# HpWang-whu/RoReg

Measured on AMD Instinct MI355X. Metric: pair-registrations/sec, higher is better.
Workload: dtype f32 (every f32 operand enters the fp16 matrix cores as hi + lo fp16 under a per-keypoint power-of-two block scale: <= 22 significant bits relative to a CONSERVATIVE per-keypoint bound -- measured on the extractor: the bound sits 2^2..2^6 above the keypoint's true coefficient maximum (config.f16x2_sc

## Files before the change

### include/roreg_hip.h

```cpp
#ifndef ROREG_HIP_H
#define ROREG_HIP_H

#include <stdint.h>
#include <stddef.h>

#ifdef __cplusplus
extern "C" {
#endif

#define ROREG_ABI_VERSION 6
int roreg_abi_version(void);
const char *roreg_last_error(void);

int roreg_set_group_tables(const int32_t *P_host, const int32_t *Nei_host, const double *R_host);

size_t roreg_group_conv_packed_size(int Cin, int Cout, int KS);
int roreg_group_conv_pack_weights(const float *W_host , int Cin, int Cout, int KS,
                                  float *wpack_host );
size_t roreg_group_conv_workspace_size(int B, int Cin, int Cout, int Lin, int Lout, int KS);
int roreg_group_conv(const float *x, const float *wpack, const float *bias,
                     const float *bn_scale, const float *bn_shift, const float *residual,
                     float *out, const int32_t *gather,
                     int B, int Cin, int Cout, int Lin, int Lout, int KS,
                     float *workspace, size_t workspace_floats, void *stream);
// ... 215 lines not shown
size_t roreg_irrep_gemm_tiles(int O, int B, int32_t *tiles_host);
size_t roreg_irrep_gemm_tiles_m(int O, int B, int tile_m , int32_t *tiles_host);
int roreg_irrep_gemm(const float *const *X, float *const *Out, const float *const *Add, const float *const *Wpack, int C, int O, int B,
                     const int32_t *tiles_dev, int n_tiles, void *stream);
int roreg_irrep_gemm_split(const float *const *X, float *const *Out, const float *const *Add, const void *const *Wsplit, int C, int O, int B,
                           const int32_t *tiles_dev, int n_tiles, void *stream);
int roreg_irrep_gemm_f16x2(const float *const *X, float *const *Out, const float *const *Add, const void *const *Wsplit2,
                           const float *x_bound_dev, int w_exp, const float *next_u_dev, const float *next_v_dev, float *out_bound_dev,
                           int C, int O, int B, const int32_t *tiles_dev, int n_tiles,
                           int tile_m ,
                           int x_planes , void *stream);
int roreg_gemm_persistent(int on);
int roreg_gemm_thin(int on);
int roreg_irrep_gemm_f16x2_rows(const float *const *X, float *T3r, const void *const *Wsplit2, const float *x_bound_dev, int w_exp, int C, int B, void *stream);
int roreg_gf_finish(const float *T3r, const float *x, const float *b_out, const float *role_scale , const float *role_shift ,
                    float *eqv, float *inv, float *role_out , float *eqv_ft, int B, void *stream);
int roreg_gf_finish_route(int on);
int roreg_row_bound(const void *x_spatial, int x_bf16 , const float *bn_scale, const float *bn_shift,
                    float *bound_out, int B, int C, void *stream);
int roreg_ft_nonlin(const float *Xin , const float *x_spatial, const float *bias,
                    const float *bias2, const float *bn_scale, const float *bn_shift, const float *resid_spatial,
                    float *Xout , float *out_spatial ,
                    const int32_t *g_map ,
                    int Lout , int Lvalid,
                    int B, int C, int split ,
                    const float *out_bound ,
                    float *out_rowmax ,
                    int spatial_bf16 ,
                    int out_planes ,
                    void *stream);
int roreg_ft_nonlin_packed(const float *Xin, const float *bias, const float *bn_scale, const float *bn_shift, uint32_t *out_words,
                           const int32_t *g_map, int Lout, int Lvalid, int B, int C, const float *out_bound, float *raw_col, int raw_g,
                           void *stream);
int roreg_ft_nonlin_gathered(const uint64_t *rows , const int64_t *dr , int feat_bf16, const float *bn_scale ,
                             const float *bn_shift, float *Xout, int B, const float *out_bound , int out_planes, void *stream);

typedef struct roreg_icp_grid_desc {
    double origin[3];
    double edge;
    int32_t dims[3];
    int32_t n;
    int64_t cells;
    int64_t reserved;
} roreg_icp_grid_desc;
size_t roreg_icp_grid_size(const double *lo_host, const double *hi_host, int n, double max_dist, roreg_icp_grid_desc *desc_host,
                           size_t *workspace_bytes);
int roreg_icp_grid_build(const float *points, const roreg_icp_grid_desc *desc_host, void *grid, void *workspace, size_t workspace_bytes,
                         void *stream);
typedef struct roreg_icp_task {
    const void *tgt_grid;
    const void *src_grid;
    const double *T0;
    int32_t n_src;
    int32_t slot0;
} roreg_icp_task;
size_t roreg_icp_batch_workspace(int n_tasks, long long total_slots);
int roreg_icp_batch(const roreg_icp_task *tasks, int n_tasks, const int32_t *work, int n_work, long long total_slots, double max_dist,
                    int max_iter, double tol_deg, double tol_t, double *T_out, int32_t *iters_out, int32_t *inliers_out, double *rmse_out,
                    int32_t *status_out, int32_t *assign_out, double *stats_out, void *workspace, size_t workspace_bytes, void *stream);

int roreg_icp_normals(const void *grid, double radius, int min_neighbors, double *out, void *stream);
typedef struct roreg_icp_plane_task {
    const void *tgt_grid;
    const void *src_grid;
    const double *tgt_normals;
    const double *T0;
// ... 155 lines not shown
```

### roreg_amd/_abi.py

```python
import ctypes
from ctypes import c_int, c_void_p, c_size_t, c_double, c_float, c_char_p

import numpy as np

ABI_VERSION = 6

_P = c_void_p
PROTOTYPES = {
    'roreg_abi_version': (c_int, []),
    'roreg_last_error': (c_char_p, []),
    'roreg_set_group_tables': (c_int, [_P, _P, _P]),
    'roreg_group_conv_packed_size': (c_size_t, [c_int, c_int, c_int]),
    'roreg_group_conv_pack_weights': (c_int, [_P, c_int, c_int, c_int, _P]),
    'roreg_group_conv_workspace_size': (c_size_t, [c_int, c_int, c_int, c_int, c_int, c_int]),
    'roreg_group_conv': (c_int, [_P, _P, _P, _P, _P, _P, _P, _P, c_int, c_int, c_int, c_int, c_int, c_int, _P, c_size_t, _P]),
    'roreg_group_conv_split': (c_int, [_P, _P, _P, _P, _P, _P, _P, _P, c_int, c_int, c_int, c_int, c_int, c_int, c_int, _P]),
    'roreg_group_conv_f16x2': (c_int, [_P, _P, c_int, _P, _P, _P, c_float, c_float, _P, _P, _P, _P, _P, c_int, c_int, c_int, c_int, c_int, c_int, c_int, _P]),
    'roreg_group_conv_f16x2_packed': (c_int, [_P, _P, c_int, _P, _P, _P, _P, _P, _P, c_int, c_int, c_int, c_int, c_int, c_int, c_int, _P]),
    'roreg_dense_f16x2': (c_int, [_P, _P, c_int, _P, _P, _P, c_float, c_float, _P, _P, c_int, _P, _P, c_int, c_int, c_int, _P]),
    'roreg_dense_split': (c_int, [_P, _P, _P, _P, _P, _P, c_int, _P, c_int, c_int, c_int, _P]),
    'roreg_gf_finalize': (c_int, [_P, _P, c_int, _P, c_int, _P]),
    'roreg_det_score': (c_int, [_P, _P, c_int, _P]),
    'roreg_inv_descriptor': (c_int, [_P, c_int, _P, c_int, _P]),
    'roreg_nn_search': (c_int, [_P, _P, c_int, _P, _P, c_int, c_int, _P, _P, _P, _P]),
# ... 84 lines not shown
    'roreg_pg_optimize_batch': (c_int, [_P, _P, c_int, _P, _P, _P, _P, _P, _P, _P, _P, _P, _P, _P, c_int, c_int, _P, _P, _P, _P, _P, _P, _P, _P, _P, _P, _P, c_size_t, _P]),
    'roreg_sparse_map_workspace': (c_size_t, [c_int]),
    'roreg_sparse_stride_map': (c_int, [_P, c_int, c_int, _P, c_int, _P, _P, _P, _P, _P, c_size_t, _P]),
    'roreg_sparse_kernel_map': (c_int, [_P, c_int, _P, c_int, c_int, c_int, _P, _P, _P, c_size_t, _P]),
    'roreg_sparse_conv': (c_int, [_P, c_int, c_int, c_int, _P, c_int, c_int, _P, c_int, _P, _P, _P, c_int, c_int, _P, c_int, _P]),
    'roreg_sparse_l2norm': (c_int, [_P, c_int, c_int, _P, _P]),
    'roreg_group_feature_assemble': (c_int, [_P, c_int, c_int, _P, _P, c_int, c_int, c_int, _P, c_int, _P, _P]),
    'roreg_sc2_workspace': (c_size_t, [ctypes.c_longlong, ctypes.c_longlong, ctypes.c_longlong, _P]),
    'roreg_sc2_hypotheses_batch': (c_int, [_P, c_int, ctypes.c_longlong, ctypes.c_longlong, ctypes.c_longlong, c_int, c_int, c_double, c_int, _P, _P, _P, _P, c_size_t, _P]),
    'roreg_fpfh_spfh_workspace': (c_size_t, [c_int]),
    'roreg_fpfh_features_workspace': (c_size_t, [c_int]),
    'roreg_fpfh_orient': (c_int, [_P, c_int, _P, _P, _P, _P]),
    'roreg_fpfh_spfh': (c_int, [_P, c_int, _P, c_double, _P, _P, _P, c_size_t, _P]),
    'roreg_fpfh_features': (c_int, [_P, c_int, _P, _P, c_double, _P, _P, _P, c_size_t, _P]),
    'roreg_fpfh_match_workspace': (c_size_t, [ctypes.c_longlong, c_int, _P]),
    'roreg_fpfh_match_batch': (c_int, [_P, c_int, c_int, c_int, ctypes.c_longlong, _P, _P, _P, _P, _P, _P, _P, c_size_t, _P]),
    'roreg_grid_knn': (c_int, [_P, c_int, c_int, c_double, _P, _P, c_int, _P, _P, _P, _P, _P]),
    'roreg_cluster_workspace': (c_size_t, [c_int]),
    'roreg_grid_dbscan': (c_int, [_P, c_int, c_double, c_int, _P, _P, _P, _P, _P, c_size_t, _P]),
    'roreg_profile_enable': (c_int, [c_int]),
    'roreg_profile_read': (c_int, [c_int, _P, _P]),
    'roreg_set_fourier_tables': (c_int, [_P]),
    'roreg_mt_shuffle_prefix': (c_int, [_P, c_int, _P, c_int, c_int, _P, c_int]),
    'roreg_mt_stream_shuffle_prefix': (c_int, [_P, _P, _P, c_int, c_int, _P]),
    'roreg_irrep_gemm_tiles': (c_size_t, [c_int, c_int, _P]),
    'roreg_irrep_gemm_tiles_m': (c_size_t, [c_int, c_int, c_int, _P]),
    'roreg_irrep_gemm': (c_int, [_P, _P, _P, _P, c_int, c_int, c_int, _P, c_int, _P]),
    'roreg_irrep_gemm_split': (c_int, [_P, _P, _P, _P, c_int, c_int, c_int, _P, c_int, _P]),
    'roreg_irrep_gemm_f16x2': (c_int, [_P, _P, _P, _P, _P, c_int, _P, _P, _P, c_int, c_int, c_int, _P, c_int, c_int, c_int, _P]),
    'roreg_row_bound': (c_int, [_P, c_int, _P, _P, _P, c_int, c_int, _P]),
    'roreg_ft_nonlin': (c_int, [_P, _P, _P, _P, _P, _P, _P, _P, _P, _P, c_int, c_int, c_int, c_int, c_int, _P, _P, c_int, c_int, _P]),
    'roreg_ft_nonlin_packed': (c_int, [_P, _P, _P, _P, _P, _P, c_int, c_int, c_int, c_int, _P, _P, c_int, _P]),
    'roreg_ft_nonlin_gathered': (c_int, [_P, _P, c_int, _P, _P, _P, c_int, _P, c_int, _P]),
}


_RANSAC_TASK = np.dtype([('keys0', np.uint64), ('keys1', np.uint64), ('matches', np.uint64), ('w', np.uint64), ('Trans', np.uint64),
                         ('hyp_rows', np.uint64), ('M', np.int32), ('H', np.int32), ('koff', np.int64)])

_MATCH_TASK = np.dtype([('desc0', np.uint64), ('desc1', np.uint64), ('rows0', np.uint64), ('rows1', np.uint64), ('m0', np.int32), ('m1', np.int32)])

_GATHER_TASK = np.dtype([('src', np.uint64), ('rows', np.uint64), ('dst', np.uint64), ('n', np.int32), ('pad', np.int32)])

_LT_TASK = np.dtype([('before0', np.uint64), ('before1', np.uint64), ('after0', np.uint64), ('after1', np.uint64), ('keys0', np.uint64),
                     ('keys1', np.uint64), ('matches', np.uint64), ('sel', np.uint64), ('n', np.int32), ('pad', np.int32), ('off', np.int64),
                     ('coef0', np.uint64), ('coef1', np.uint64)])

_ICP_GRID_DESC = np.dtype([('origin', np.float64, 3), ('edge', np.float64), ('dims', np.int32, 3), ('n', np.int32), ('cells', np.int64),
                           ('reserved', np.int64)])

_ICP_TASK = np.dtype([('tgt_grid', np.uint64), ('src_grid', np.uint64), ('T0', np.uint64), ('n_src', np.int32), ('slot0', np.int32)])

_ICP_PLANE_TASK = np.dtype([('tgt_grid', np.uint64), ('src_grid', np.uint64), ('tgt_normals', np.uint64), ('T0', np.uint64), ('n_src', np.int32),
                            ('slot0', np.int32)])

_ICP_GICP_TASK = np.dtype([('tgt_grid', np.uint64), ('src_grid', np.uint64), ('tgt_normals', np.uint64), ('src_normals', np.uint64), ('T0', np.uint64),
                           ('epsilon', np.float64), ('n_src', np.int32), ('slot0', np.int32)])

_ICP_LOSS = {'huber': 1, 'cauchy': 2, 'gm': 3, 'tukey': 4}
_ICP_PLANE_ROBUST_TASK = np.dtype(_ICP_PLANE_TASK.descr + [('scale', np.float64), ('loss', np.int32), ('reserved', np.int32)])
_ICP_GICP_ROBUST_TASK = np.dtype(_ICP_GICP_TASK.descr + [('scale', np.float64), ('loss', np.int32), ('reserved', np.int32)])
assert _ICP_PLANE_ROBUST_TASK.itemsize == 56 and _ICP_GICP_ROBUST_TASK.itemsize == 72

_PG_GRAPH = np.dtype([('node0', np.int32), ('n_nodes', np.int32), ('edge0', np.int32), ('n_edges', np.int32), ('act0', np.int32), ('n_act', np.int32),
                      ('anchor', np.int32), ('reserved0', np.int32), ('h0', np.int64), ('tau', np.float64), ('lambda0', np.float64),
                      ('tol_t', np.float64), ('tol_rot', np.float64), ('tol_cost', np.float64), ('reserved1', np.float64)])
# ... 8 lines not shown
```

### roreg_amd/_hip_fourier.py

```python
import os
from ctypes import c_void_p

import numpy as np
import torch

from . import hip as _core
from .hip import HipError, _check, _feat, _ptr, _stream, lib

__all__ = ['DenseSplitLayer', 'IRREP_DIMS', 'IRREP_OFFSETS', '_bf16_split3', '_keypoint_of_columns', '_ptr_array', '_res_ptr', '_tile_cache', 'bf16_split3_frags', 'bf16_split3_pack', 'bound_exp', 'coef_pitch', 'coef_size', 'coef_views', 'dense_split', 'ensure_fourier', 'f16_scale_exp', 'f16_split2_frags', 'f16_split2_pack', 'frag_pack', 'ft_nonlin', 'ft_nonlin_gathered', 'ft_nonlin_packed', 'gemm_persistent', 'gemm_thin', 'gf_finish', 'gf_finish_rows', 'gf_finish_usable', 'group_conv_split_pack', 'irrep_gemm', 'irrep_gemm_rows', 'next_bound', 'next_bound_spatial', 'pack_coefs_f16x2', 'row_bound', 'unpack_coefs_f16x2', 'words_to_planes']


_fourier_ready = False
IRREP_DIMS = (1, 3, 3, 4, 5)
IRREP_OFFSETS = (0, 1, 10, 19, 35, 60)


def ensure_fourier():
    global _fourier_ready
    if not _fourier_ready:
        from .fourier import group_fourier
        F = np.ascontiguousarray(group_fourier().F, np.float32)
        _check(lib().roreg_set_fourier_tables(F.ctypes.data), 'roreg_set_fourier_tables')
        _fourier_ready = True


def _ptr_array(views):
    arr = (c_void_p * 5)(*[c_void_p(v.data_ptr()) for v in views])
    return arr


def coef_pitch(B):
    return (int(B) + 31) // 32 * 32


def coef_size(C, B):
    return 60 * C * coef_pitch(B)


def coef_views(buf, C, B):
    Bp = coef_pitch(B)
    return [buf[IRREP_OFFSETS[r] * C * Bp:IRREP_OFFSETS[r + 1] * C * Bp].view(IRREP_DIMS[r] * C, IRREP_DIMS[r] * Bp) for r in range(5)]

# ... 159 lines not shown
        o.copy_(w.view(torch.float32))
    return out, bound


def words_to_planes(X_words, C, B):
    w = X_words.contiguous().view(torch.int32).view(-1, 2, 16)
    hi = (w & 0xffff).to(torch.int16).transpose(1, 2); lo = (w >> 16).to(torch.int16).transpose(1, 2)
    return torch.cat([hi.reshape(-1, 32), lo.reshape(-1, 32)], 1).contiguous().view(torch.float32).view(-1)


def unpack_coefs_f16x2(X_words, bound, C, B):
    Bp = coef_pitch(B)
    e = bound_exp(bound)
    out = torch.empty_like(X_words)
    for r, (v, o) in enumerate(zip(coef_views(X_words, C, B), coef_views(out, C, B))):
        kp = _keypoint_of_columns(IRREP_DIMS[r], Bp)
        w = v.view(torch.int32)
        hi = (w & 0xffff).to(torch.int16).view(torch.float16).float()
        lo = (w >> 16).to(torch.int16).view(torch.float16).float()
        o.copy_(torch.ldexp(hi + lo, -e[kp][None, :]))
    return out


def next_bound_spatial(bn, bias):
    scale, shift = bn
    sc = scale.detach().double().abs().cpu(); sh = shift.detach().double().abs().cpu()
    b = bias.detach().double().cpu()
    k = 1.0 + 2.0 ** -9
    u = (np.sqrt(60.0) * k) * sc
    v = k * (sc * b.abs() + sh) + 1e-30
    return u.float().cuda().contiguous(), v.float().cuda().contiguous()


def ft_nonlin_packed(B, C, coef_in, bias, bn, out_bound, g_map=None, Lout=60, Lvalid=60, raw_g=None):
    ensure_fourier()
    dev = coef_in.device
    if coef_in.numel() != coef_size(C, B) or out_bound.numel() != coef_pitch(B):
        raise HipError('ft_nonlin_packed: coef_in / out_bound sizes')
    words = torch.empty((B, C, Lout if g_map is not None else 60), dtype=torch.int32, device=dev)
    raw = torch.empty((B, C), dtype=torch.float32, device=dev) if raw_g is not None else None
    scale, shift = bn if bn is not None else (None, None)
    _check(lib().roreg_ft_nonlin_packed(_ptr(coef_in, torch.float32), _ptr(bias), _ptr(scale), _ptr(shift), _ptr(words), _ptr(g_map, torch.int32),
                                        int(Lout), int(Lvalid), B, C, _ptr(out_bound, torch.float32), _ptr(raw), int(raw_g or 0), _stream()),
           'roreg_ft_nonlin_packed')
    return words, raw


def next_bound(bn, bias, bias2=None):
    scale, shift = bn
    sc = scale.detach().double().abs().cpu(); sh = shift.detach().double().abs().cpu()
    b = bias.detach().double().cpu() + (bias2.detach().double().cpu() if bias2 is not None else 0.0)
    k = 1.0 + 2.0 ** -9
    u = (60.0 * k) * sc
    v = (np.sqrt(60.0) * k) * (sc * b.abs() + sh) + 1e-30
    return u.float().cuda().contiguous(), v.float().cuda().contiguous()


def ft_nonlin(B, C, coef_in=None, x_spatial=None, bias=None, bias2=None, bn=None, resid_spatial=None, spatial_out=False,
              g_map=None, Lout=60, Lvalid=60, split=False, out_bound=None, want_rowmax=False, planes=False):
    ensure_fourier()
    dev = (coef_in if coef_in is not None else x_spatial).device
    if spatial_out:
        out = torch.empty((B, C, Lout if g_map is not None else 60), dtype=torch.float32, device=dev); xout = None; osp = _ptr(out)
    else:
        out = torch.empty(coef_size(C, B), dtype=torch.float32, device=dev); xout = _ptr(out); osp = None
    scale, shift = bn if bn is not None else (None, None)
    if want_rowmax and not spatial_out:
        raise HipError('ft_nonlin: want_rowmax goes with spatial_out')
    amax = torch.zeros(B, dtype=torch.float32, device=dev) if want_rowmax else None
# ... 123 lines not shown
```

### roreg_amd/csrc/fourier.hip

```cpp
#include "common.h"
#include "primitives.h"
#include <algorithm>
#include <atomic>
#include <cmath>
#include <cstdlib>
#include <type_traits>
#include <utility>
#include <vector>

namespace {

constexpr int NIRR = 5;

struct GemmDescs {
    const float *X[NIRR];
    float *Out[NIRR];
    const float *Add[NIRR];
    const float4 *W[NIRR];
    int K[NIRR], M[NIRR], Mpad[NIRR], N[NIRR];
};

__device__ __forceinline__ void lds_dma16(const void *src, void *dst) {
    __builtin_amdgcn_global_load_lds((const __attribute__((address_space(1))) void *)src, (__attribute__((address_space(3))) void *)dst, 16, 0, 0);
}
// ... 1984 lines not shown
                    unsigned *dst = reinterpret_cast<unsigned *>(const_cast<char *>(slot_ptr(ic, p.Xout, c, tb)));
                    if (kPS.kind[S] != 2 || h == 0) __builtin_nontemporal_store(word, dst);
                });
            } else {
                const int tb = tbi;
                static_for<32>([&](auto ic) {
                    constexpr int S = decltype(ic)::value, t = S / 16, r = S % 16;
                    float *dst = reinterpret_cast<float *>(const_cast<char *>(slot_ptr(ic, p.Xout, c, tb)));
                    if (kPS.kind[S] != 2 || h == 0) __builtin_nontemporal_store(o[t][r], dst);
                });
            }
        }
    };
    if (wave_global < n_tiles) {
        const int last = wave_global + ((n_tiles - 1 - wave_global) / n_waves) * n_waves;
        float cb[NCV + 1];
        GDesc da{0u, 0u, 0}, db{0u, 0u, 0};
        if constexpr (GATHER) {
            da = load_desc(wave_global);
            db = load_desc(min(wave_global + n_waves, last));
            load_rows_gathered(wave_global, da, cn);
        } else {
            load_coefs(wave_global, cn);
        }
        __builtin_amdgcn_s_waitcnt(0x0F70);
        for (int tile = wave_global; tile <= last; tile += 2 * n_waves) {
            const int t1 = min(tile + n_waves, last), t2 = min(tile + 2 * n_waves, last), t3 = min(tile + 3 * n_waves, last);
            process(tile, t1, cn, cb, t2, db, da);
            process(t1, t2, cb, cn, t3, da, db);
        }
    }
}

#undef OFF_OF
#undef OFF_Q

struct GfFinishParams {
    const float *T3r;
    const float *x;
    const float *b_out;
    const float *role_scale, *role_shift;
    float *eqv, *inv, *role_out, *eqv_ft;
    const f16x8 *A1h, *A2h;
    int f_exp, B;
};

__global__ __launch_bounds__(256, 2) void gf_finish_kernel(GfFinishParams p) {
    constexpr int NA = 4 * 2 * 2 * 64 * 4;
    extern __shared__ __attribute__((aligned(16))) float gf_smem[];
    float *sA1 = gf_smem, *sA2 = gf_smem + NA, *sT = gf_smem + 2 * NA, *sRole = sT + 4 * 32 * 65;
    const int lane = threadIdx.x & 63, jn = lane & 31, h = lane >> 5;
    {
        const float *g1 = reinterpret_cast<const float *>(p.A1h), *g2 = reinterpret_cast<const float *>(p.A2h);
        for (int i = threadIdx.x; i < NA; i += 256) { sA1[i] = g1[i]; sA2[i] = g2[i]; }
        if (threadIdx.x < 128) sRole[threadIdx.x] = p.role_scale ? (threadIdx.x < 64 ? p.role_scale[threadIdx.x] : p.role_shift[threadIdx.x - 64]) : 0.f;
    }
    __syncthreads();
    const f16x8 *sA1h = reinterpret_cast<const f16x8 *>(sA1), *sA2h = reinterpret_cast<const f16x8 *>(sA2);
    const int wave_global = __builtin_amdgcn_readfirstlane((blockIdx.x * 256 + threadIdx.x) >> 6);
    const int n_waves = gridDim.x * 4;
    const int B = p.B;
    const bool act = lane < ROREG_G;
    const float bo = p.b_out[jn] + 0.f;
    float *ti = sT + (threadIdx.x >> 6) * (32 * 65);

    auto load = [&](int b, float (&cv)[32], float (&xv)[32]) {
// ... 138 lines not shown
                if constexpr (kPS.qb[S] < ROREG_G) ti[jn * 65 + kPS.qb[S]] = o[S / 16][S % 16];
            });
        }
        ROREG_LDS_DONE();
        float *fo = p.eqv_ft + (size_t)b * (ROREG_F * ROREG_G) + lane;
#pragma unroll
        for (int c8 = 0; c8 < 4; ++c8) {
            float tv[8];
#pragma unroll
            for (int q = 0; q < 8; ++q) tv[q] = ti[(c8 * 8 + q) * 65 + lane];
#pragma unroll
            for (int q = 0; q < 8; ++q)
                if (act) fo[(c8 * 8 + q) * ROREG_G] = tv[q];
        }
        ROREG_LDS_DONE();
    };
#undef ROREG_LDS_DONE
    if (wave_global < B) {
        const int last = wave_global + ((B - 1 - wave_global) / n_waves) * n_waves;
        float ca[32], xa[32], cb[32], xb[32];
        load(wave_global, ca, xa);
        __builtin_amdgcn_s_waitcnt(0x0F70);
        for (int b = wave_global; b <= last; b += 2 * n_waves) {
            const int b1 = min(b + n_waves, last), b2 = min(b + 2 * n_waves, last);
            process(b, b1, ca, xa, cb, xb);
            process(b1, b2, cb, xb, ca, xa);
        }
    }
}

float *g_A1 = nullptr, *g_A2 = nullptr;
uint16_t *g_A1s = nullptr, *g_A2s = nullptr, *g_A1h = nullptr, *g_A2h = nullptr;
int g_f_exp = 0;

}

extern "C" int roreg_set_fourier_tables(const float *F_host ) {
    ROREG_REQUIRE(F_host, "roreg_set_fourier_tables: null table");
    static float A1[30 * 2 * 64], A2[32 * 2 * 64];
    for (int s = 0; s < 30; ++s)
        for (int tile = 0; tile < 2; ++tile)
            for (int lane = 0; lane < 64; ++lane) {
                const int qq = 2 * s + (lane >> 5), g = tile * 32 + (lane & 31);
                A1[(s * 2 + tile) * 64 + lane] = g < 60 ? F_host[qq * 60 + g] : 0.f;
            }
    for (int t = 0; t < 2; ++t)
        for (int r = 0; r < 16; ++r)
            for (int tile = 0; tile < 2; ++tile)
                for (int lane = 0; lane < 64; ++lane) {
                    const int qq = slot_out_q(tile * 32 + (lane & 31)), g = cd_row32(r, lane >> 5, t * 32);
                    A2[((t * 16 + r) * 2 + tile) * 64 + lane] = (qq < 60 && g < 60) ? F_host[qq * 60 + g] : 0.f;
                }
    if (!g_A1) {
        if (hipMalloc(&g_A1, sizeof(A1)) != hipSuccess || hipMalloc(&g_A2, sizeof(A2)) != hipSuccess) {
            roreg::set_error("roreg_set_fourier_tables: hipMalloc failed");
            return 1;
        }
    }
    if (hipMemcpy(g_A1, A1, sizeof(A1), hipMemcpyHostToDevice) != hipSuccess || hipMemcpy(g_A2, A2, sizeof(A2), hipMemcpyHostToDevice) != hipSuccess) {
        roreg::set_error("roreg_set_fourier_tables: hipMemcpy failed");
        return 1;
    }
    static uint16_t A1s[4 * 2 * 3 * 64 * 8], A2s[4 * 2 * 3 * 64 * 8];
    auto split3_host = [](float x, uint16_t out[3]) {
        float rem = x;
        for (int sp = 0; sp < 3; ++sp) {
// ... 38 lines not shown
    int fex = 0;
    (void)std::frexp(fmx, &fex);
    g_f_exp = fmx > 0.f ? 14 - fex : 0;
    auto f2h = [](float x) -> uint16_t {
        _Float16 hv = (_Float16)x;
        uint16_t b; memcpy(&b, &hv, 2);
        return b;
    };
    auto h2f = [](uint16_t b) -> float { _Float16 hv; memcpy(&hv, &b, 2); return (float)hv; };
    for (int st = 0; st < 4; ++st)
        for (int tile = 0; tile < 2; ++tile)
            for (int lane = 0; lane < 64; ++lane)
                for (int e = 0; e < 8; ++e) {
                    const int j = lane & 31, h = lane >> 5;
                    const int q1 = 16 * st + 8 * h + e, g1 = tile * 32 + j;
                    const float f1 = (q1 < 60 && g1 < 60) ? std::ldexp(F_host[q1 * 60 + g1], g_f_exp) : 0.f;
                    const int r = 8 * (st & 1) + e, q2 = slot_out_q(tile * 32 + j), g2 = cd_row32(r, h, 32 * (st >> 1));
                    const float f2 = (q2 < 60 && g2 < 60) ? std::ldexp(F_host[q2 * 60 + g2], g_f_exp) : 0.f;
                    const uint16_t h1 = f2h(f1), h2 = f2h(f2);
                    const size_t hi_at = ((((size_t)st * 2 + tile) * 2 + 0) * 64 + lane) * 8 + e, lo_at = hi_at + 64 * 8;
                    A1h[hi_at] = h1; A1h[lo_at] = f2h(f1 - h2f(h1));
                    A2h[hi_at] = h2; A2h[lo_at] = f2h(f2 - h2f(h2));
                }
    if (!g_A1h) {
        if (hipMalloc(&g_A1h, sizeof(A1h)) != hipSuccess || hipMalloc(&g_A2h, sizeof(A2h)) != hipSuccess) {
            roreg::set_error("roreg_set_fourier_tables: hipMalloc failed");
            return 1;
        }
    }
    if (hipMemcpy(g_A1h, A1h, sizeof(A1h), hipMemcpyHostToDevice) != hipSuccess || hipMemcpy(g_A2h, A2h, sizeof(A2h), hipMemcpyHostToDevice) != hipSuccess) {
        roreg::set_error("roreg_set_fourier_tables: hipMemcpy failed");
        return 1;
    }
    return 0;
}

extern "C" size_t roreg_irrep_gemm_tiles_m(int O, int B, int tile_m, int32_t *tiles_host);
extern "C" size_t roreg_irrep_gemm_tiles(int O, int B, int32_t *tiles_host ) { return roreg_irrep_gemm_tiles_m(O, B, 128, tiles_host); }

extern "C" size_t roreg_irrep_gemm_tiles_m(int O, int B, int tile_m , int32_t *tiles_host) {
    static const int dims[5] = {1, 3, 3, 4, 5};
    struct Block { int r, mg, ng, cost; };
    std::vector<Block> blocks;
    for (int r = 4; r >= 0; --r) {
        const int d = dims[r];
        const int mts = round_up(d * O, tile_m) / tile_m, nts = (d * B + 255) / 256;
        for (int ng = 0; ng * 8 < nts; ++ng)
            for (int mg = 0; mg * 8 < mts; ++mg) {
                const int a = std::min(8, mts - mg * 8), b = std::min(8, nts - ng * 8);
                blocks.push_back({r, mg, ng, a * b * d});
            }
    }
    std::stable_sort(blocks.begin(), blocks.end(), [](const Block &x, const Block &y) { return x.cost > y.cost; });
    std::vector<std::vector<int>> stream(8);
    long long load[8] = {0, 0, 0, 0, 0, 0, 0, 0};
    for (const Block &bk : blocks) {
        int k = 0;
        for (int q = 1; q < 8; ++q)
            if (load[q] < load[k]) k = q;
        load[k] += bk.cost;
        const int d = dims[bk.r];
        const int mts = round_up(d * O, tile_m) / tile_m, nts = (d * B + 255) / 256;
        for (int nt = bk.ng * 8; nt < std::min(nts, bk.ng * 8 + 8); ++nt)
            for (int mt = bk.mg * 8; mt < std::min(mts, bk.mg * 8 + 8); ++mt) {
                stream[k].push_back(bk.r); stream[k].push_back(mt); stream[k].push_back(nt);
            }
// ... 231 lines not shown
    p.bias = bias; p.bias2 = bias2; p.bn_scale = bn_scale; p.bn_shift = bn_shift; p.A1 = g_A1; p.A2 = g_A2;
    p.A1s = reinterpret_cast<const bf16x8 *>(g_A1s); p.A2s = reinterpret_cast<const bf16x8 *>(g_A2s); p.out_bound = out_bound; p.out_rowmax = out_rowmax; p.x_bf16 = spatial_bf16;
    p.A1h = reinterpret_cast<const f16x8 *>(g_A1h); p.A2h = reinterpret_cast<const f16x8 *>(g_A2h); p.f_exp = g_f_exp;
    p.B = B; p.Bp = (B + 31) / 32 * 32; p.C = C; p.tiles_per_c = (B + 31) / 32;
    p.out_planes = out_planes;
    ROREG_REQUIRE((unsigned long long)C * p.Bp * 20ull < (1ull << 32), "roreg_ft_nonlin: C * round_up(B, 32) must stay below 2^32 / 20 (32-bit lane offsets)");
    ROREG_REQUIRE(!out_planes || (split == 2 && Xout), "roreg_ft_nonlin: out_planes is a layout of the fp16 x 2 coefficient output");
    const long long n_tiles = (long long)C * p.tiles_per_c;
    hipStream_t s = roreg::as_stream(stream);
    roreg::ProfScope prof(roreg::PROF_FT_NONLIN, s);
    const bool in_sp = x_spatial != nullptr, out_sp = out_spatial != nullptr;
    if (in_sp && out_sp) { roreg::set_error("roreg_ft_nonlin: spatial -> spatial is not a transform"); return 2; }
    ROREG_REQUIRE(split != 2 || out_sp || out_bound, "roreg_ft_nonlin: split = 2 writes the coefficients as fp16 hi/lo pairs and needs out_bound");
    ROREG_REQUIRE(!spatial_bf16 || in_sp || resid_spatial, "roreg_ft_nonlin: spatial_bf16 refers to x_spatial / resid_spatial");
    ROREG_REQUIRE(!out_rowmax || out_sp, "roreg_ft_nonlin: out_rowmax goes with a group-domain output");
    ROREG_REQUIRE(split >= 0 && split <= 2, "roreg_ft_nonlin: split must be 0 (f32 MFMA), 1 (bf16 x 3) or 2 (fp16 x 2)");
    if (split == 2) {
        if (in_sp) launch_ft<ft_nonlin_kernel<true, false, 2, 4, 1>>(p, n_tiles, s);
        else if (!out_sp) launch_ft<ft_nonlin_kernel<false, false, 2, 4, 1>>(p, n_tiles, s);
        else launch_ft<ft_nonlin_kernel<false, true, 2, 4, 1>>(p, n_tiles, s);
    } else if (split == 1) {
        if (in_sp) launch_ft<ft_nonlin_kernel<true, false, 3, 4, 1>>(p, n_tiles, s);
        else if (!out_sp) launch_ft<ft_nonlin_kernel<false, false, 3, 4, 1>>(p, n_tiles, s);
        else launch_ft<ft_nonlin_kernel<false, true, 3, 4, 1>>(p, n_tiles, s);
    } else {
        if (in_sp) launch_ft<ft_nonlin_kernel<true, false, 0, 4, 1>>(p, n_tiles, s);
        else if (!out_sp) launch_ft<ft_nonlin_kernel<false, false, 0, 4, 1>>(p, n_tiles, s);
        else launch_ft<ft_nonlin_kernel<false, true, 0, 4, 1>>(p, n_tiles, s);
    }
    ROREG_CHECK_LAUNCH("roreg_ft_nonlin");
    return 0;
}

extern "C" int roreg_ft_nonlin_packed(const float *Xin, const float *bias, const float *bn_scale, const float *bn_shift, uint32_t *out_words,
                                      const int32_t *g_map, int Lout, int Lvalid, int B, int C, const float *out_bound, float *raw_col, int raw_g,
                                      void *stream) {
    ROREG_REQUIRE(g_A1 && g_A2, "roreg_ft_nonlin_packed: roreg_set_fourier_tables has not been called");
    ROREG_REQUIRE(Xin && out_words && out_bound && B > 0 && C > 0 && C <= 512 && (bn_scale == nullptr) == (bn_shift == nullptr), "roreg_ft_nonlin_packed: bad arguments");
    ROREG_REQUIRE(!g_map || (Lout >= Lvalid && Lvalid > 0 && Lout <= 64), "roreg_ft_nonlin_packed: bad Lout/Lvalid");
    ROREG_REQUIRE(!raw_col || (raw_g >= 0 && raw_g < ROREG_G), "roreg_ft_nonlin_packed: raw_g out of range");
    NonlinParams p;
    memset(&p, 0, sizeof(p));
    p.Xin = Xin; p.out_spatial = reinterpret_cast<float *>(out_words);
    p.g_map = g_map; p.Lout = g_map ? Lout : ROREG_G; p.Lvalid = g_map ? Lvalid : ROREG_G;
    p.bias = bias; p.bn_scale = bn_scale; p.bn_shift = bn_shift; p.A1 = g_A1; p.A2 = g_A2;
    p.A1s = reinterpret_cast<const bf16x8 *>(g_A1s); p.A2s = reinterpret_cast<const bf16x8 *>(g_A2s);
    p.A1h = reinterpret_cast<const f16x8 *>(g_A1h); p.A2h = reinterpret_cast<const f16x8 *>(g_A2h); p.f_exp = g_f_exp;
    p.out_bound = out_bound; p.sp_pack = 1; p.raw_col = raw_col; p.raw_g = raw_g;
    p.B = B; p.Bp = (B + 31) / 32 * 32; p.C = C; p.tiles_per_c = (B + 31) / 32;
    ROREG_REQUIRE((unsigned long long)C * p.Bp * 20ull < (1ull << 32), "roreg_ft_nonlin_packed: C * round_up(B, 32) must stay below 2^32 / 20 (32-bit lane offsets)");
    hipStream_t s = roreg::as_stream(stream);
    roreg::ProfScope prof(roreg::PROF_FT_NONLIN, s);
    launch_ft<ft_nonlin_kernel<false, true, 2, 4, 1>>(p, (long long)C * p.tiles_per_c, s);
    ROREG_CHECK_LAUNCH("roreg_ft_nonlin_packed");
    return 0;
}

extern "C" int roreg_ft_nonlin_gathered(const uint64_t *rows, const int64_t *dr, int feat_bf16, const float *bn_scale, const float *bn_shift, float *Xout,
                                        int B, const float *out_bound, int out_planes, void *stream) {
    ROREG_REQUIRE(g_A1 && g_A2, "roreg_ft_nonlin_gathered: roreg_set_fourier_tables has not been called");
    ROREG_REQUIRE(roreg::group_tables().ready, "roreg_ft_nonlin_gathered: group tables not set");
    ROREG_REQUIRE(rows && dr && Xout && out_bound && B > 0 && (bn_scale == nullptr) == (bn_shift == nullptr), "roreg_ft_nonlin_gathered: bad arguments");
    constexpr int C = 4 * ROREG_F;
    ROREG_REQUIRE((long long)60 * C * B < (1ll << 40), "roreg_ft_nonlin_gathered: tensor too large");
    NonlinParams p;
    memset(&p, 0, sizeof(p));
    p.Xout = Xout; p.Lout = ROREG_G; p.Lvalid = ROREG_G;
    p.bn_scale = bn_scale; p.bn_shift = bn_shift; p.A1 = g_A1; p.A2 = g_A2;
    p.A1s = reinterpret_cast<const bf16x8 *>(g_A1s); p.A2s = reinterpret_cast<const bf16x8 *>(g_A2s);
    p.A1h = reinterpret_cast<const f16x8 *>(g_A1h); p.A2h = reinterpret_cast<const f16x8 *>(g_A2h); p.f_exp = g_f_exp;
    p.out_bound = out_bound; p.x_bf16 = feat_bf16; p.out_planes = out_planes;
    p.g_rows = reinterpret_cast<const roreg::LtRow *>(rows); p.g_dr = dr; p.g_P8 = roreg::group_tables().P8;
    p.B = B; p.Bp = (B + 31) / 32 * 32; p.C = C; p.tiles_per_c = (B + 31) / 32;
    ROREG_REQUIRE((unsigned long long)C * p.Bp * 20ull < (1ull << 32), "roreg_ft_nonlin_gathered: 128 * round_up(B, 32) must stay below 2^32 / 20 (32-bit lane offsets)");
    hipStream_t s = roreg::as_stream(stream);
    roreg::ProfScope prof(roreg::PROF_FT_NONLIN, s);
    launch_ft<ft_nonlin_kernel<true, false, 2, 4, 1, false, true>>(p, (long long)C * p.tiles_per_c, s);
    ROREG_CHECK_LAUNCH("roreg_ft_nonlin_gathered");
    return 0;
}

extern "C" int roreg_feat_coefs(const void *x, int x_bf16, float *out, int B, int C, int split, void *stream) {
    if (B == 0) return 0;
    ROREG_REQUIRE(g_A1 && g_A2, "roreg_feat_coefs: roreg_set_fourier_tables has not been called");
    ROREG_REQUIRE(x && out && B > 0 && C > 0 && C <= 512 && split >= 0 && split <= 2, "roreg_feat_coefs: bad arguments");
    NonlinParams p;
// ... 53 lines not shown
```

Measured before the change: 1126.

## Add specialized inverse-Fourier packed kernel for ET column map with permuted table

Adds a dedicated persistent kernel for ft_nonlin_packed when a 48-column group map is used. The inverse transform table is pre-permuted on the host so the map's gather folds into the matrix product, which skips work on dropped columns and drops the generic map lookup. The kernel double-buffers coefficient loads across tiles and can pair two tiles per store. It is enabled by default via a route switch and adds host-side table caching keyed on the map and a table generation counter.

```diff
diff --git a/include/roreg_hip.h b/include/roreg_hip.h
--- a/include/roreg_hip.h
+++ b/include/roreg_hip.h
@@ -271,6 +271,10 @@
 int roreg_ft_nonlin_packed(const float *Xin, const float *bias, const float *bn_scale, const float *bn_shift, uint32_t *out_words,
                            const int32_t *g_map, int Lout, int Lvalid, int B, int C, const float *out_bound, float *raw_col, int raw_g,
                            void *stream);
+int roreg_et_ift_permute_table(const uint16_t *A1h, const int32_t *map , uint16_t *out);
+int roreg_set_et_ift_map(const int32_t *map_host , const int32_t *map_dev );
+int roreg_et_ift_route(int on);
+int roreg_et_ift_usable(const int32_t *g_map, int Lout, int Lvalid, int has_raw, int raw_g, int C);
 int roreg_ft_nonlin_gathered(const uint64_t *rows , const int64_t *dr , int feat_bf16, const float *bn_scale ,
                              const float *bn_shift, float *Xout, int B, const float *out_bound , int out_planes, void *stream);
 
diff --git a/roreg_amd/_abi.py b/roreg_amd/_abi.py
--- a/roreg_amd/_abi.py
+++ b/roreg_amd/_abi.py
@@ -140,6 +140,10 @@
     'roreg_ft_nonlin': (c_int, [_P, _P, _P, _P, _P, _P, _P, _P, _P, _P, c_int, c_int, c_int, c_int, c_int, _P, _P, c_int, c_int, _P]),
     'roreg_ft_nonlin_packed': (c_int, [_P, _P, _P, _P, _P, _P, c_int, c_int, c_int, c_int, _P, _P, c_int, _P]),
     'roreg_ft_nonlin_gathered': (c_int, [_P, _P, c_int, _P, _P, _P, c_int, _P, c_int, _P]),
+    'roreg_et_ift_permute_table': (c_int, [_P, _P, _P]),
+    'roreg_set_et_ift_map': (c_int, [_P, _P]),
+    'roreg_et_ift_route': (c_int, [c_int]),
+    'roreg_et_ift_usable': (c_int, [_P, c_int, c_int, c_int, c_int, c_int]),
 }
 
 
diff --git a/roreg_amd/_hip_fourier.py b/roreg_amd/_hip_fourier.py
--- a/roreg_amd/_hip_fourier.py
+++ b/roreg_amd/_hip_fourier.py
@@ -7,7 +7,7 @@
 from . import hip as _core
 from .hip import HipError, _check, _feat, _ptr, _stream, lib
 
-__all__ = ['DenseSplitLayer', 'IRREP_DIMS', 'IRREP_OFFSETS', '_bf16_split3', '_keypoint_of_columns', '_ptr_array', '_res_ptr', '_tile_cache', 'bf16_split3_frags', 'bf16_split3_pack', 'bound_exp', 'coef_pitch', 'coef_size', 'coef_views', 'dense_split', 'ensure_fourier', 'f16_scale_exp', 'f16_split2_frags', 'f16_split2_pack', 'frag_pack', 'ft_nonlin', 'ft_nonlin_gathered', 'ft_nonlin_packed', 'gemm_persistent', 'gemm_thin', 'gf_finish', 'gf_finish_rows', 'gf_finish_usable', 'group_conv_split_pack', 'irrep_gemm', 'irrep_gemm_rows', 'next_bound', 'next_bound_spatial', 'pack_coefs_f16x2', 'row_bound', 'unpack_coefs_f16x2', 'words_to_planes']
+__all__ = ['DenseSplitLayer', 'IRREP_DIMS', 'IRREP_OFFSETS', '_bf16_split3', '_keypoint_of_columns', '_ptr_array', '_res_ptr', '_tile_cache', 'bf16_split3_frags', 'bf16_split3_pack', 'bound_exp', 'coef_pitch', 'coef_size', 'coef_views', 'dense_split', 'ensure_fourier', 'et_ift', 'et_ift_register', 'f16_scale_exp', 'f16_split2_frags', 'f16_split2_pack', 'frag_pack', 'ft_nonlin', 'ft_nonlin_gathered', 'ft_nonlin_packed', 'gemm_persistent', 'gemm_thin', 'gf_finish', 'gf_finish_rows', 'gf_finish_usable', 'group_conv_split_pack', 'irrep_gemm', 'irrep_gemm_rows', 'next_bound', 'next_bound_spatial', 'pack_coefs_f16x2', 'row_bound', 'unpack_coefs_f16x2', 'words_to_planes']
 
 
 _fourier_ready = False
@@ -233,9 +233,29 @@
     return u.float().cuda().contiguous(), v.float().cuda().contiguous()
 
 
+et_ift = _GemmSwitch('roreg_et_ift_route', int,
+                     """`with hip.et_ift(True | False | 2):` -- whether ft_nonlin_packed's launch form in ET (a column map, 48 columns) runs on et_ift_packed_kernel
+    (roreg_et_ift_route; ROREG_ET_IFT in the environment sets the initial value) or on the generic transform kernel.  Same bits either way -- tests and A/B
+    measurements.""")
+
+_et_ift_map = None
+
+
+def et_ift_register(g_map):
+    global _et_ift_map
+    if _et_ift_map is not None and _et_ift_map[0] is g_map and _et_ift_map[1] == g_map._version:
+        return
+    _et_ift_map = None
+    host = np.ascontiguousarray(g_map.detach().cpu().numpy(), np.int32)
+    _check(lib().roreg_set_et_ift_map(host.ctypes.data, _ptr(g_map, torch.int32)), 'roreg_set_et_ift_map')
+    _et_ift_map = (g_map, g_map._version)
+
+
 def ft_nonlin_packed(B, C, coef_in, bias, bn, out_bound, g_map=None, Lout=60, Lvalid=60, raw_g=None):
     ensure_fourier()
     dev = coef_in.device
+    if g_map is not None and Lout == 48 and g_map.numel() == 60 and g_map.dtype == torch.int32 and g_map.is_contiguous():
+        et_ift_register(g_map)
     if coef_in.numel() != coef_size(C, B) or out_bound.numel() != coef_pitch(B):
         raise HipError('ft_nonlin_packed: coef_in / out_bound sizes')
     words = torch.empty((B, C, Lout if g_map is not None else 60), dtype=torch.int32, device=dev)
diff --git a/roreg_amd/csrc/fourier.hip b/roreg_amd/csrc/fourier.hip
--- a/roreg_amd/csrc/fourier.hip
+++ b/roreg_amd/csrc/fourier.hip
@@ -2040,6 +2040,196 @@
     }
 }
 
+struct EtIftParams {
+    const float *Xin;
+    uint32_t *out;
+    const float *bias, *bn_scale, *bn_shift;
+    const f16x8 *A1c;
+    const float *out_bound;
+    float *raw_col;
+    int raw_e, raw_h;
+    int f_exp, B, Bp, C, Lvalid;
+};
+
+template <bool PAIR>
+__global__ __launch_bounds__(256, PAIR ? 2 : 3) void et_ift_packed_kernel(EtIftParams p) {
+    constexpr int NT = 256, LOUT = 48, NEL = 24;
+    constexpr int PITCH = PAIR ? 2 * LOUT + 1 : LOUT + 1;
+    const int lane = threadIdx.x & 63;
+    const int jn = lane & 31, h = lane >> 5;
+    const int wave_global = __builtin_amdgcn_readfirstlane((blockIdx.x * NT + threadIdx.x) >> 6);
+    const int n_waves = gridDim.x * 4;
+    const int B = p.B, C = p.C;
+    const int n_tiles = C * ((B + 31) >> 5);
+    constexpr int NA1 = 4 * 2 * 2 * 64 * 4;
+    __shared__ __attribute__((aligned(16))) float sA1[NA1];
+    __shared__ float sT[4 * 32 * PITCH];
+    __shared__ float sBias[512], sScale[512], sShift[512];
+    {
+        const float *g1 = reinterpret_cast<const float *>(p.A1c);
+        for (int i = threadIdx.x; i < NA1; i += NT) sA1[i] = g1[i];
+    }
+    for (int i = threadIdx.x; i < C; i += NT) {
+        sBias[i] = (p.bias ? p.bias[i] : 0.f) + 0.f;
+        sScale[i] = p.bn_scale ? p.bn_scale[i] : 1.f;
+        sShift[i] = p.bn_shift ? p.bn_shift[i] : 0.f;
+    }
+    __syncthreads();
+    const f16x8 *sA1h = reinterpret_cast<const f16x8 *>(sA1);
+    const size_t Bp = (size_t)p.Bp;
+    const size_t hmask = (size_t)0 - (size_t)h;
+    float *const tbuf = sT + (threadIdx.x >> 6) * (32 * PITCH);
+    float *const twr = tbuf + jn * PITCH + 4 * h;
+    const bool bn = p.bn_scale != nullptr;
+
+    auto load_coefs = [&](int tile, float (&dst)[33]) {
+        const int c = tile % C, tb = tile / C;
+        dst[32] = p.out_bound[tb * 32 + jn];
+        static_for<32>([&](auto ic) {
+            constexpr int st = decltype(ic)::value / 8, e = decltype(ic)::value % 8;
+            constexpr int q0 = 16 * st + e, q1 = 16 * st + 8 + e;
+            if constexpr (q1 < ROREG_G) dst[st * 8 + e] = __builtin_nontemporal_load(p.Xin + OFF_OF(q0, q1, c, tb) + jn);
+            else dst[st * 8 + e] = __builtin_nontemporal_load(p.Xin + OFF_Q(q0, c, tb) + jn);
+        });
+    };
+    auto table_mma = [&](const f16x8 *a, const f16x8 (&b)[2], f32x16 c) {
+        f16x8 av[2];
+#pragma unroll
+        for (int pl = 0; pl < 2; ++pl) av[pl] = a[64 * pl];
+        return split_mma<2>(av, b, c);
+    };
+    auto column_scale = [&](float mx, float &xscale, float &oscale) {
+        mx = fmaxf(mx, __shfl_xor(mx, 32));
+        int e = 0;
+        if (mx > 0.f && mx < __builtin_inff()) { int ex; (void)frexpf(mx, &ex); e = 14 - ex; }
+        xscale = ldexpf(1.f, e); oscale = ldexpf(1.f, -(e + p.f_exp));
+    };
+    auto store_rows = [&](int c, int tbi) {
+        asm volatile("s_waitcnt lgkmcnt(0)" ::: "memory");
+        const int b0 = tbi * 32;
+        const size_t ostep = (size_t)C * LOUT;
+        if constexpr (!PAIR) {
+            const int lc = lane < LOUT ? lane : LOUT - 1;
+            if (b0 + 32 <= B) {
+                uint32_t *ob = p.out + ((size_t)b0 * C + c) * LOUT + lane;
+#pragma unroll
+                for (int g8 = 0; g8 < 4; ++g8) {
+                    float tv[8];
+#pragma unroll
+                    for (int q = 0; q < 8; ++q) tv[q] = tbuf[(g8 * 8 + q) * PITCH + lc];
+#pragma unroll
+                    for (int q = 0; q < 8; ++q)
+                        if (lane < LOUT) ob[(size_t)(g8 * 8 + q) * ostep] = lane < p.Lvalid ? __float_as_uint(tv[q]) : 0u;
+                }
+            } else {
+                for (int bl = 0; bl < 32 && b0 + bl < B; ++bl)
+                    if (lane < LOUT) p.out[((size_t)(b0 + bl) * C + c) * LOUT + lane] = lane < p.Lvalid ? __float_as_uint(tbuf[bl * PITCH + lc]) : 0u;
+            }
+        } else {
+            const bool live_a = (lane < LOUT ? lane : lane - LOUT) < p.Lvalid, live_b = 16 + jn < p.Lvalid;
+            if (b0 + 32 <= B) {
+                uint32_t *oa = p.out + ((size_t)b0 * C + c) * LOUT + lane;
+                uint32_t *obb = p.out + ((size_t)(b0 + h) * C + c) * LOUT + 64 + jn;
+                const float *ra = tbuf + lane, *rb = tbuf + h * PITCH + 64 + jn;
+#pragma unroll
+                for (int g8 = 0; g8 < 4; ++g8) {
+                    float ta[8], tc[4];
+#pragma unroll
+                    for (int q = 0; q < 8; ++q) ta[q] = ra[(g8 * 8 + q) * PITCH];
+#pragma unroll
+                    for (int q = 0; q < 4; ++q) tc[q] = rb[(g8 * 8 + 2 * q) * PITCH];
+#pragma unroll
+                    for (int q = 0; q < 8; ++q) oa[(size_t)(g8 * 8 + q) * ostep] = live_a ? __float_as_uint(ta[q]) : 0u;
+#pragma unroll
+                    for (int q = 0; q < 4; ++q) obb[(size_t)(g8 * 8 + 2 * q) * ostep] = live_b ? __float_as_uint(tc[q]) : 0u;
+                }
+            } else {
+                for (int bl = 0; bl < 32 && b0 + bl < B; ++bl) {
+                    uint32_t *orow = p.out + ((size_t)(b0 + bl) * C + c) * LOUT;
+                    orow[lane] = live_a ? __float_as_uint(tbuf[bl * PITCH + lane]) : 0u;
+                    if (h == 0) orow[64 + jn] = live_b ? __float_as_uint(tbuf[bl * PITCH + 64 + jn]) : 0u;
+                }
+            }
+        }
+        asm volatile("s_waitcnt lgkmcnt(0)" ::: "memory");
+    };
+    auto process = [&](int tile, int next_tile, float (&cv)[33], float (&cnext)[33], auto slotc) {
+        constexpr int SLOT = decltype(slotc)::value;
+        asm volatile("" ::: "memory");
+        const int c = tile % C, tbi = tile / C;
+        const int b = tbi * 32 + jn;
+        const bool valid = b < B;
+        const int bb = valid ? b : B - 1;
+        f32x16 v[2];
+        load_coefs(next_tile, cnext);
+        __builtin_amdgcn_sched_barrier(0);
+#pragma unroll
+        for (int t = 0; t < 2; ++t)
+#pragma unroll
+            for (int r = 0; r < 16; ++r) v[t][r] = 0.f;
+        float mx = 0.f;
+#pragma unroll
+        for (int s = 0; s < 32; ++s) mx = fmaxf(mx, ((16 * (s >> 3) + 8 + (s & 7) < ROREG_G || h == 0) ? fabsf(cv[s]) : 0.f));
+        float xsc, osc;
+        column_scale(mx, xsc, osc);
+#pragma unroll
+        for (int st = 0; st < 4; ++st) {
+            float x8[8];
+#pragma unroll
+            for (int e = 0; e < 8; ++e) x8[e] = (16 * st + 8 + e < ROREG_G || h == 0) ? cv[st * 8 + e] : 0.f;
+            f16x8 bh, bl;
+            split2(x8, xsc, bh, bl);
+            const f16x8 bq[2] = {bh, bl};
+            v[0] = table_mma(sA1h + ((st * 2 + 0) * 2) * 64 + lane, bq, v[0]);
+            v[1] = table_mma(sA1h + ((st * 2 + 1) * 2) * 64 + lane, bq, v[1]);
+        }
+        const float bsum = sBias[c], sc = sScale[c], sh = sShift[c];
+        const float pk_scale = ldexpf(1.f, bound_exp(cv[32]));
+        float rawv = 0.f;
+        static_for<NEL>([&](auto ec) {
+            constexpr int E = decltype(ec)::value, t = E / 16, r = E % 16;
+            float x = v[t][r] * osc + bsum;
+            rawv = E == p.raw_e ? x : rawv;
+            if (bn) x = fmaxf(fmaf(x, sc, sh), 0.f);
+            const float xs = x * pk_scale;
+            const _Float16 h1 = (_Float16)xs;
+            const _Float16 l1 = (_Float16)(xs - (float)h1);
+            twr[SLOT * LOUT + 32 * t + (r & 3) + 8 * (r >> 2)] =
+                __uint_as_float((unsigned)__builtin_bit_cast(unsigned short, h1) | ((unsigned)__builtin_bit_cast(unsigned short, l1) << 16));
+        });
+        if (p.raw_col && h == p.raw_h && valid) p.raw_col[(size_t)bb * C + c] = rawv;
+        if constexpr (!PAIR) store_rows(c, tbi);
+    };
+    using S0 = std::integral_constant<int, 0>;
+    using S1 = std::integral_constant<int, PAIR ? 1 : 0>;
+    float cn[33], cb[33];
+    if constexpr (!PAIR) {
+        if (wave_global < n_tiles) {
+            const int last = wave_global + ((n_tiles - 1 - wave_global) / n_waves) * n_waves;
+            load_coefs(wave_global, cn);
+            __builtin_amdgcn_s_waitcnt(0x0F70);
+            for (int tile = wave_global; tile <= last; tile += 2 * n_waves) {
+                const int t1 = min(tile + n_waves, last), t2 = min(tile + 2 * n_waves, last);
+                process(tile, t1, cn, cb, S0{});
+                process(t1, t2, cb, cn, S1{});
+            }
+        }
+    } else {
+        const int n_units = n_tiles >> 1;
+        if (wave_global < n_units) {
+            const int last = wave_global + ((n_units - 1 - wave_global) / n_waves) * n_waves;
+            load_coefs(2 * wave_global, cn);
+            __builtin_amdgcn_s_waitcnt(0x0F70);
+            for (int u = wave_global; u <= last; u += n_waves) {
+                const int un = min(u + n_waves, last);
+                process(2 * u, 2 * u + 1, cn, cb, S0{});
+                process(2 * u + 1, 2 * un, cb, cn, S1{});
+                store_rows((2 * u) % C, (2 * u) / C);
+            }
+        }
+    }
+}
+
 #undef OFF_OF
 #undef OFF_Q
 
@@ -2244,6 +2434,7 @@
 float *g_A1 = nullptr, *g_A2 = nullptr;
 uint16_t *g_A1s = nullptr, *g_A2s = nullptr, *g_A1h = nullptr, *g_A2h = nullptr;
 int g_f_exp = 0;
+int g_tables_gen = 0;
 
 }
 
@@ -2348,6 +2539,7 @@
         roreg::set_error("roreg_set_fourier_tables: hipMemcpy failed");
         return 1;
     }
+    ++g_tables_gen;
     return 0;
 }
 
@@ -2645,6 +2837,95 @@
     return 0;
 }
 
+extern "C" int roreg_et_ift_permute_table(const uint16_t *A1h , const int32_t *map , uint16_t *out ) {
+    if (!A1h || !map || !out) return -1;
+    int src[64], live = 0;
+    for (int i = 0; i < 64; ++i) src[i] = -1;
+    for (int g = 0; g < ROREG_G; ++g) {
+        if (map[g] < 0) continue;
+        if (map[g] >= 48 || src[map[g]] >= 0) return -1;
+        src[map[g]] = g; ++live;
+    }
+    for (int st = 0; st < 4; ++st)
+        for (int tile = 0; tile < 2; ++tile)
+            for (int pl = 0; pl < 2; ++pl)
+                for (int lane = 0; lane < 64; ++lane) {
+                    const int g = src[tile * 32 + (lane & 31)];
+                    uint16_t *o = out + ((((size_t)st * 2 + tile) * 2 + pl) * 64 + lane) * 8;
+                    if (g < 0) { memset(o, 0, 16); continue; }
+                    memcpy(o, A1h + ((((size_t)st * 2 + g / 32) * 2 + pl) * 64 + ((lane & 32) | (g % 32))) * 8, 16);
+                }
+    return live;
+}
+
+namespace {
+struct EtIftMap {
+    int32_t map[ROREG_G];
+    int live;
+    int gen;
+    uint16_t *table;
+};
+std::vector<EtIftMap> g_et_maps;
+int g_et_cur = -1;
+const int32_t *g_et_cur_dev = nullptr;
+}
+static GemmSwitch g_et_ift{"ROREG_ET_IFT", 2, 2};
+extern "C" int roreg_et_ift_route(int on) { return g_et_ift.set(on); }
+
+extern "C" int roreg_set_et_ift_map(const int32_t *map_host , const int32_t *map_dev ) {
+    ROREG_REQUIRE(g_A1h, "roreg_set_et_ift_map: roreg_set_fourier_tables has not been called");
+    ROREG_REQUIRE(map_host && map_dev, "roreg_set_et_ift_map: null map");
+    g_et_cur = -1; g_et_cur_dev = nullptr;
+    for (size_t i = 0; i < g_et_maps.size(); ++i)
+        if (g_et_maps[i].gen == g_tables_gen && !memcmp(g_et_maps[i].map, map_host, sizeof(g_et_maps[i].map))) { g_et_cur = (int)i; break; }
+    if (g_et_cur < 0) {
+        constexpr size_t n = 4 * 2 * 2 * 64 * 8;
+        std::vector<uint16_t> A1h(n), perm(n);
+        if (hipMemcpy(A1h.data(), g_A1h, n * sizeof(uint16_t), hipMemcpyDeviceToHost) != hipSuccess) {
+            roreg::set_error("roreg_set_et_ift_map: hipMemcpy failed");
+            return 1;
+        }
+        EtIftMap m;
+        memcpy(m.map, map_host, sizeof(m.map));
+        m.live = roreg_et_ift_permute_table(A1h.data(), map_host, perm.data());
+        m.table = nullptr; m.gen = g_tables_gen;
+        bool dense = m.live > 0;
+        for (int g = 0; g < ROREG_G && dense; ++g) dense = map_host[g] < m.live;
+        if (dense) {
+            if (hipMalloc(&m.table, n * sizeof(uint16_t)) != hipSuccess || hipMemcpy(m.table, perm.data(), n * sizeof(uint16_t), hipMemcpyHostToDevice) != hipSuccess) {
+                roreg::set_error("roreg_set_et_ift_map: hipMalloc / hipMemcpy failed");
+                return 1;
+            }
+        }
+        g_et_maps.push_back(m);
+        g_et_cur = (int)g_et_maps.size() - 1;
+    }
+    g_et_cur_dev = map_dev;
+    return 0;
+}
+
+extern "C" int roreg_et_ift_usable(const int32_t *g_map, int Lout, int Lvalid, int has_raw, int raw_g, int C) {
+    const int route = g_et_ift.get();
+    if (!route || !g_map || g_map != g_et_cur_dev || g_et_cur < 0) return 0;
+    const EtIftMap &m = g_et_maps[g_et_cur];
+    if (!m.table || m.gen != g_tables_gen || Lout != 48 || Lvalid != m.live || C <= 0 || C > 512) return 0;
+    if (has_raw && (raw_g < 0 || raw_g >= ROREG_G || m.map[raw_g] < 0)) return 0;
+    return route == 2 && C % 2 == 0 ? 2 : 1;
+}
+
+template <bool PAIR>
+static void launch_et_ift(const EtIftParams &p, hipStream_t s) {
+    static const int resident = [] {
+        int per_cu = 0, dev = 0, cus = 256;
+        if (hipOccupancyMaxActiveBlocksPerMultiprocessor(&per_cu, et_ift_packed_kernel<PAIR>, 256, 0) != hipSuccess || per_cu < 1) per_cu = 2;
+        if (hipGetDevice(&dev) == hipSuccess) (void)hipDeviceGetAttribute(&cus, hipDeviceAttributeMultiprocessorCount, dev);
+        return per_cu * cus;
+    }();
+    const long long units = (long long)p.C * ((p.B + 31) / 32) / (PAIR ? 2 : 1);
+    const long long want = (units + 3) / 4, cap = (long long)resident * 4;
+    hipLaunchKernelGGL(et_ift_packed_kernel<PAIR>, dim3((unsigned)(want > cap ? cap : want)), dim3(256), 0, s, p);
+}
+
 extern "C" int roreg_ft_nonlin_packed(const float *Xin, const float *bias, const float *bn_scale, const float *bn_shift, uint32_t *out_words,
                                       const int32_t *g_map, int Lout, int Lvalid, int B, int C, const float *out_bound, float *raw_col, int raw_g,
                                       void *stream) {
@@ -2664,7 +2945,19 @@
     ROREG_REQUIRE((unsigned long long)C * p.Bp * 20ull < (1ull << 32), "roreg_ft_nonlin_packed: C * round_up(B, 32) must stay below 2^32 / 20 (32-bit lane offsets)");
     hipStream_t s = roreg::as_stream(stream);
     roreg::ProfScope prof(roreg::PROF_FT_NONLIN, s);
-    launch_ft<ft_nonlin_kernel<false, true, 2, 4, 1>>(p, (long long)C * p.tiles_per_c, s);
+    if (const int form = roreg_et_ift_usable(g_map, Lout, Lvalid, raw_col != nullptr, raw_g, C)) {
+        const EtIftMap &m = g_et_maps[g_et_cur];
+        EtIftParams q;
+        memset(&q, 0, sizeof(q));
+        q.Xin = Xin; q.out = out_words; q.bias = bias; q.bn_scale = bn_scale; q.bn_shift = bn_shift;
+        q.A1c = reinterpret_cast<const f16x8 *>(m.table); q.out_bound = out_bound; q.raw_col = raw_col;
+        const int pos = raw_col ? m.map[raw_g] : -1;
+        q.raw_e = raw_col ? 16 * (pos >> 5) + (pos & 3) + 4 * ((pos & 31) >> 3) : -1; q.raw_h = raw_col ? (pos >> 2) & 1 : 0;
+        q.f_exp = g_f_exp; q.B = B; q.Bp = p.Bp; q.C = C; q.Lvalid = Lvalid;
+        if (form == 2) launch_et_ift<true>(q, s); else launch_et_ift<false>(q, s);
+    } else {
+        launch_ft<ft_nonlin_kernel<false, true, 2, 4, 1>>(p, (long long)C * p.tiles_per_c, s);
+    }
     ROREG_CHECK_LAUNCH("roreg_ft_nonlin_packed");
     return 0;
 }
```

Result: no change. 1136, median of 6 (+0.9%).
